# waiwnf/pilotguru

Hardware: AMD Instinct MI355X
Metric: frames/sec ORB extract+match, 1080p @ 2000 kp/frame (higher is better)
Workload: dtype u8

## Files before the change

pilotguru_amd/csrc/describe.hip:

```cpp
#include "pgorb_internal.h"

struct PgGauss7 { int k0, k1, k2, k3; };
constexpr PgGauss7 PG_G7 = {18, 34, 49, 55};

#define DH_N 37

struct PgDescTab { uint32_t mom[5 * 64]; uint32_t btab[3 * 64 * 4]; int8_t pat[64 * 4 * 4]; };
constexpr PgDescTab pg_make_desc_tab()
{
    constexpr int umax[16] = {15, 15, 15, 15, 14, 14, 14, 13, 13, 12, 11, 10, 9, 8, 6, 3};
    constexpr int8_t p[256 * 4] = {
#include "orb_pattern31.inc"
    };
    constexpr int K[7] = {PG_G7.k0, PG_G7.k1, PG_G7.k2, PG_G7.k3, PG_G7.k2, PG_G7.k1, PG_G7.k0};
    PgDescTab t = {};
    for (int r = 0; r < 31; r++)
        for (int q = 0; q < 9; q++) {
            const int vy = r - 15, dmax = umax[vy < 0 ? -vy : vy];
            uint32_t wu = 0;
            for (int k = 0; k < 4; k++) {
                const int ux = 4 * (q + 1) + k - 21;
                if ((ux < 0 ? -ux : ux) <= dmax) wu |= (uint32_t)(ux + 16) << (8 * k);
            }
            t.mom[r * 9 + q] = wu;
        }
    for (int cb = 0; cb < 3; cb++)
        for (int l = 0; l < 64; l++)
            for (int j = 0; j < 16; j++) {
                const int k = 16 * (l >> 4) + j, n = 16 * cb + (l & 15), d = k - n;
                const uint32_t v = (d >= 0 && d <= 6 && n < DH_N) ? (uint32_t)K[d] : 0u;
                t.btab[(cb * 64 + l) * 4 + j / 4] |= v << (8 * (j % 4));
            }
    for (int l = 0; l < 64; l++)
        for (int r = 0; r < 4; r++)
            for (int k = 0; k < 4; k++) t.pat[(l * 4 + r) * 4 + k] = p[(64 * r + l) * 4 + k];
    return t;
}
__device__ static const __attribute__((aligned(16))) PgDescTab pg_desc_tab = pg_make_desc_tab();

#define DW_R 21
#define DW_N 43
#define DW_PITCH 48
#define DH_PITCH 40
#define DB_PITCH 40

__device__ __forceinline__ int pg_reflect101(int p, int n)
{
    if (n == 1) return 0;
    while (p < 0 || p >= n) p = (p < 0) ? -p : 2 * (n - 1) - p;
    return p;
}

__device__ __forceinline__ float pg_fast_atan2(float y, float x)
{
    const float scale = (float)(180 / 3.1415926535897932384626433832795);
    const float p1 = 0.9997878412794807f * scale, p3 = -0.3258083974640975f * scale;
    const float p5 = 0.1555786518463281f * scale, p7 = -0.04432655554792128f * scale;
    const float eps = (float)2.2204460492503131e-16;
    const float ax = fabsf(x), ay = fabsf(y);
    float a, c, c2;
    if (ax >= ay) {
        c = __fdiv_rn(ay, __fadd_rn(ax, eps));
        c2 = __fmul_rn(c, c);
        a = __fmul_rn(__fadd_rn(__fmul_rn(__fadd_rn(__fmul_rn(__fadd_rn(__fmul_rn(p7, c2), p5), c2), p3), c2), p1), c);
    } else {
        c = __fdiv_rn(ax, __fadd_rn(ay, eps));
        c2 = __fmul_rn(c, c);
        a = __fsub_rn(90.f, __fmul_rn(__fadd_rn(__fmul_rn(__fadd_rn(__fmul_rn(__fadd_rn(__fmul_rn(p7, c2), p5), c2), p3), c2), p1), c));
    }
    if (x < 0) a = __fsub_rn(180.f, a);
    if (y < 0) a = __fsub_rn(360.f, a);
    return a;
}

__device__ __forceinline__ void pg_sincos_f(float angle, float* s_out, float* c_out)
{
    const double INV_PIO2 = 0.63661977236758138243;
    const double PIO2_HI = 1.57079632673412561417e+00;
    const double PIO2_LO = 6.07710050650619224932e-11;
    const double x = (double)angle;
    const double kd = floor(__dadd_rn(__dmul_rn(x, INV_PIO2), 0.5));
    const double r = __dsub_rn(__dsub_rn(x, __dmul_rn(kd, PIO2_HI)), __dmul_rn(kd, PIO2_LO));
    const double r2 = __dmul_rn(r, r);
    double ps = -1.0 / 355687428096000.0;
    ps = __dadd_rn(__dmul_rn(ps, r2), 1.0 / 1307674368000.0);
    ps = __dsub_rn(__dmul_rn(ps, r2), 1.0 / 6227020800.0);
    ps = __dadd_rn(__dmul_rn(ps, r2), 1.0 / 39916800.0);
    ps = __dsub_rn(__dmul_rn(ps, r2), 1.0 / 362880.0);
    ps = __dadd_rn(__dmul_rn(ps, r2), 1.0 / 5040.0);
    ps = __dsub_rn(__dmul_rn(ps, r2), 1.0 / 120.0);
    ps = __dadd_rn(__dmul_rn(ps, r2), 1.0 / 6.0);
    const double sn = __dsub_rn(r, __dmul_rn(__dmul_rn(r, r2), ps));
    double pc = -1.0 / 6402373705728000.0;
    pc = __dadd_rn(__dmul_rn(pc, r2), 1.0 / 20922789888000.0);
    pc = __dsub_rn(__dmul_rn(pc, r2), 1.0 / 87178291200.0);
    pc = __dadd_rn(__dmul_rn(pc, r2), 1.0 / 479001600.0);
    pc = __dsub_rn(__dmul_rn(pc, r2), 1.0 / 3628800.0);
    pc = __dadd_rn(__dmul_rn(pc, r2), 1.0 / 40320.0);
    pc = __dsub_rn(__dmul_rn(pc, r2), 1.0 / 720.0);
    pc = __dadd_rn(__dmul_rn(pc, r2), 1.0 / 24.0);
    pc = __dsub_rn(__dmul_rn(pc, r2), 0.5);
    const double cs = __dadd_rn(1.0, __dmul_rn(r2, pc));
    const int k = (int)((long long)kd & 3);
    const double s = (k == 0) ? sn : (k == 1) ? cs : (k == 2) ? -sn : -cs;
    const double c = (k == 0) ? cs : (k == 1) ? -sn : (k == 2) ? -cs : sn;
    *s_out = (float)s;
    *c_out = (float)c;
}

__device__ __forceinline__ int pg_wave_sum(int x)
{
    int v = x;
    v += __builtin_amdgcn_update_dpp(0, v, 0x111, 0xf, 0xf, true);
    v += __builtin_amdgcn_update_dpp(0, v, 0x112, 0xf, 0xf, true);
    v += __builtin_amdgcn_update_dpp(0, v, 0x114, 0xf, 0xf, true);
    v += __builtin_amdgcn_update_dpp(0, v, 0x118, 0xf, 0xf, true);
    v += __builtin_amdgcn_update_dpp(0, v, 0x142, 0xa, 0xf, false);
    v += __builtin_amdgcn_update_dpp(0, v, 0x143, 0xc, 0xf, false);
    return __builtin_amdgcn_readlane(v, 63);
}


typedef __attribute__((address_space(1))) const void* pg_gptr_t;
typedef __attribute__((address_space(3))) void* pg_lptr_t;
typedef unsigned short pg_us2 __attribute__((ext_vector_type(2)));
typedef int pg_v4i __attribute__((ext_vector_type(4)));
#define PG_GLOBAL __attribute__((address_space(1)))
typedef PG_GLOBAL const uint8_t* pg_gbytes_t;

__device__ __forceinline__ int pg_blur_at(const uint32_t* hT, int Y, int X, bool tieEven)
{
    constexpr PgGauss7 G = PG_G7;
    const pg_us2 K01 = {(unsigned short)G.k0, (unsigned short)G.k1}, K23 = {(unsigned short)G.k2, (unsigned short)G.k3},
                 K45 = {(unsigned short)G.k2, (unsigned short)G.k1};
    const uint32_t* s = hT + (Y >> 1) * 40 + X;
    const uint32_t p0 = s[0], p1 = s[40], p2 = s[80], p3 = s[120];
    const uint32_t sh = (uint32_t)(Y & 1) << 4;
    const uint32_t a0 = __builtin_amdgcn_alignbit(p1, p0, sh), a1 = __builtin_amdgcn_alignbit(p2, p1, sh),
                   a2 = __builtin_amdgcn_alignbit(p3, p2, sh), last = (p3 >> sh) & 0xFFFFu;
    uint32_t C = __builtin_amdgcn_udot2(__builtin_bit_cast(pg_us2, a0), K01, (uint32_t)G.k0 * last, false);
    C = __builtin_amdgcn_udot2(__builtin_bit_cast(pg_us2, a1), K23, C, false);
    C = __builtin_amdgcn_udot2(__builtin_bit_cast(pg_us2, a2), K45, C, false);
    int v = (int)((C + 32768u) >> 16);
    if (tieEven && (C & 0xFFFFu) == 0x8000u) v &= ~1;
    return min(v, 255);
}

#define PG_WAVE_SYNC() do { __builtin_amdgcn_fence(__ATOMIC_RELEASE, "wavefront"); __builtin_amdgcn_wave_barrier(); \
                            __builtin_amdgcn_fence(__ATOMIC_ACQUIRE, "wavefront"); } while (0)

struct PgDescArgs {
    const int32_t* kpCount;  const PgSelRec* sel;  int64_t selFrame;  pgorb_keypoint* kps;
    uint8_t* desc;  int32_t* n_out;  int32_t nlevels, tieMode, cap_per_frame, slotBeg;
    int32_t slotEnd, writeTotal, slotsPerXcd, pad[5];
};
static_assert(sizeof(PgDescArgs) == 96 && sizeof(PgDescArgs) <= 128, "one s_load_dwordx16 + one s_load_dwordx8");

__global__ __launch_bounds__(64) void k_describe(const PgDescArgs KA)
{
    __shared__ __attribute__((aligned(16))) uint32_t hbuf[22 * DH_PITCH];
    uint8_t* raw = reinterpret_cast<uint8_t*>(hbuf);

    const int lane = threadIdx.x;
    const uint32_t frame = blockIdx.y;
    typedef int32_t pg_i32x16 __attribute__((ext_vector_type(16)));
    typedef uint32_t pg_u32x16 __attribute__((ext_vector_type(16)));
    typedef uint32_t pg_u32x8 __attribute__((ext_vector_type(8)));
    pg_gbytes_t tb = (pg_gbytes_t)(const void*)&pg_desc_tab;
    asm volatile("" : "+s"(tb));
    const uint32_t o4 = 4u * (uint32_t)lane, o16 = 16u * (uint32_t)lane;
    uint32_t mt[5];
#pragma unroll
    for (int it = 0; it < 5; it++) mt[it] = *(const PG_GLOBAL uint32_t*)(tb + (offsetof(PgDescTab, mom) + 256 * it) + o4);
    pg_v4i Bop[3];
#pragma unroll
    for (int cb = 0; cb < 3; cb++) Bop[cb] = *(const PG_GLOBAL pg_v4i*)(tb + (offsetof(PgDescTab, btab) + 1024 * cb) + o16);
    const pg_v4i pat = *(const PG_GLOBAL pg_v4i*)(tb + offsetof(PgDescTab, pat) + o16);
    pg_u32x16 a0;
    pg_u32x8 a1;
    asm volatile("s_load_dwordx16 %0, %2, 0x0\n\ts_load_dwordx8 %1, %2, 0x40\n\ts_waitcnt lgkmcnt(0)"
                 : "=&s"(a0), "=&s"(a1) : "s"(__builtin_amdgcn_kernarg_segment_ptr()) : "memory");
#define PG_A64(T, v, k) reinterpret_cast<T>((uintptr_t)(((uint64_t)(v)[(k) + 1] << 32) | (v)[k]))
    const int32_t* kpCount = PG_A64(const int32_t*, a0, 0);
    const PgSelRec* sel = PG_A64(const PgSelRec*, a0, 2);
    const int64_t selFrame = (int64_t)(((uint64_t)a0[5] << 32) | a0[4]);
    pgorb_keypoint* kps = PG_A64(pgorb_keypoint*, a0, 6);
    uint8_t* desc = PG_A64(uint8_t*, a0, 8);
    int32_t* n_out = PG_A64(int32_t*, a0, 10);
#undef PG_A64
    const int nlevels = (int)a0[12], tieMode = (int)a0[13], cap_per_frame = (int)a0[14], slotBeg = (int)a0[15];
    const int slotEnd = (int)a1[0], writeTotal = (int)a1[1], slotsPerXcd = (int)a1[2];
    const int slot = slotBeg + (int)(blockIdx.x & 7) * slotsPerXcd + (int)(blockIdx.x >> 3);
    const int32_t* kpc = kpCount + frame * PG_MAXL;
    const PgSelRec* recp = sel + ((int64_t)frame * selFrame + slot);
    pg_i32x16 kc;
    pg_u32x8 rec;
    asm volatile("s_load_dwordx16 %0, %2, 0x0\n\ts_load_dwordx8 %1, %3, 0x0\n\ts_waitcnt lgkmcnt(0)" : "=&s"(kc), "=&s"(rec) : "s"(kpc), "s"(recp) : "memory");
    if (slot >= slotEnd) return;
    const int l = (int)(rec[1] >> 16) & 15;
    int total = 0, before = 0;
#pragma unroll
    for (int q = 0; q < PG_MAXL; q++) {
        const int c = kc[q];
        if (q < l) before += c;
        total += c;
    }
    if (writeTotal && blockIdx.x == 0 && lane == 0) n_out[frame] = total;
    if (rec[1] == 0xFFFFFFFFu || l >= nlevels) return;
    const uint32_t cv = rec[0];
    const int idx = before + (int)(rec[1] & 0xFFFFu);
    const int Lpitch = (int)rec[2], Lw = (int)(rec[3] & 0xFFFFu), Lh = (int)(rec[3] >> 16);
    const uint8_t* img = reinterpret_cast<const uint8_t*>((uintptr_t)(((uint64_t)rec[5] << 32) | rec[4]));
    const float Lscale = __uint_as_float(rec[6]), LpatchSize = __uint_as_float(rec[7]);
    const int x = (int)(cv & 0xFFF) + PG_EDGE, y = (int)((cv >> 12) & 0xFFF) + PG_EDGE;
    const int resp = (int)(cv >> 24);
    const int w = Lw, h = Lh;

    const int x0 = x - DW_R, y0 = y - DW_R;
    if (x0 >= 0 && y0 >= 0 && x0 + DW_PITCH <= w && y + DW_R < h) {
        const int lr = lane / 3, lq = lane - 3 * lr;
        const uint8_t* g = img + (int64_t)(y0 + lr) * Lpitch + x0 + 16 * lq;
        if (lr < 21) {
            __builtin_amdgcn_global_load_lds((pg_gptr_t)g, (pg_lptr_t)raw, 16, 0, 0);
            __builtin_amdgcn_global_load_lds((pg_gptr_t)(g + 21 * (int64_t)Lpitch), (pg_lptr_t)(raw + 21 * DW_PITCH), 16, 0, 0);
            if (lr < 1)
                __builtin_amdgcn_global_load_lds((pg_gptr_t)(g + 42 * (int64_t)Lpitch), (pg_lptr_t)(raw + 42 * DW_PITCH), 16, 0, 0);
        }
        __builtin_amdgcn_s_waitcnt(0);
    } else {
        for (int i = lane; i < DW_N * DW_PITCH; i += 64) {
            const int r = i / DW_PITCH, c = i - r * DW_PITCH;
            raw[r * DW_PITCH + c] =
                img[(int64_t)pg_reflect101(y0 + r, h) * Lpitch + pg_reflect101(x0 + c, w)];
        }
    }
    PG_WAVE_SYNC();

    int m10 = 0, m01 = 0;
#pragma unroll
    for (int it = 0; it < 5; it++) {
        const int i = lane + 64 * it;
        if (i >= 31 * 9) break;
        const int r = i / 9, q = i - r * 9;
        const uint32_t val = *reinterpret_cast<const uint32_t*>(raw + (DW_R - 15 + r) * DW_PITCH + 4 * (q + 1));
        const uint32_t wm = ((mt[it] + 0x7F7F7F7Fu) >> 7) & 0x01010101u;
        const int sv = (int)__builtin_amdgcn_udot4(val, wm, 0u, false);
        m10 += (int)__builtin_amdgcn_udot4(val, mt[it], 0u, false) - 16 * sv;
        m01 += (r - 15) * sv;
    }
    m10 = pg_wave_sum(m10);
    m01 = pg_wave_sum(m01);
    const float angle = pg_fast_atan2((float)m01, (float)m10);

    uint32_t* hT = hbuf;
    {
        constexpr int cinit = 128 * (2 * (PG_G7.k0 + PG_G7.k1 + PG_G7.k2) + PG_G7.k3);
        pg_v4i Aop[3];
#pragma unroll
        for (int rb = 0; rb < 3; rb++) {
            Aop[rb] = *reinterpret_cast<const pg_v4i*>(raw + (16 * rb + (lane & 15)) * DW_PITCH + 16 * (lane >> 4));
            Aop[rb].x ^= (int)0x80808080; Aop[rb].y ^= (int)0x80808080; Aop[rb].z ^= (int)0x80808080; Aop[rb].w ^= (int)0x80808080;
        }
        PG_WAVE_SYNC();
#pragma unroll
        for (int rb = 0; rb < 3; rb++) {
            const int pair = 8 * rb + 2 * (lane >> 4);
#pragma unroll
            for (int cb = 0; cb < 3; cb++) {
                const pg_v4i acc = __builtin_amdgcn_mfma_i32_16x16x64_i8(Aop[rb], Bop[cb], pg_v4i{cinit, cinit, cinit, cinit}, 0, 0, 0);
                const int n = 16 * cb + (lane & 15);
                if (n < DH_PITCH) {
                    if (pair < 22) hT[pair * DH_PITCH + n] = (uint32_t)acc.x | ((uint32_t)acc.y << 16);
                    if (pair + 1 < 22) hT[(pair + 1) * DH_PITCH + n] = (uint32_t)acc.z | ((uint32_t)acc.w << 16);
                }
            }
        }
    }
    PG_WAVE_SYNC();
    const int wvec = w & ~3;

    const float factorPI = (float)(3.1415926535897932384626433832795 / 180.f);
    float a, b;
    pg_sincos_f(__fmul_rn(angle, factorPI), &b, &a);
    unsigned long long bits[4];
#pragma unroll
    for (int r = 0; r < 4; r++) {
        const uint32_t pw = (uint32_t)pat[r];
        const float px0 = (float)(int8_t)(pw & 0xFF), py0 = (float)(int8_t)((pw >> 8) & 0xFF);
        const float px1 = (float)(int8_t)((pw >> 16) & 0xFF), py1 = (float)(int8_t)(pw >> 24);
        const int r0 = __float2int_rn(__fadd_rn(__fmul_rn(px0, b), __fmul_rn(py0, a)));
        const int c0 = __float2int_rn(__fsub_rn(__fmul_rn(px0, a), __fmul_rn(py0, b)));
        const int r1 = __float2int_rn(__fadd_rn(__fmul_rn(px1, b), __fmul_rn(py1, a)));
        const int c1 = __float2int_rn(__fsub_rn(__fmul_rn(px1, a), __fmul_rn(py1, b)));
        const int t0 = pg_blur_at(hT, 18 + r0, 18 + c0, tieMode == 0 && x + c0 < wvec);
        const int t1 = pg_blur_at(hT, 18 + r1, 18 + c1, tieMode == 0 && x + c1 < wvec);
        bits[r] = __ballot(t0 < t1);
    }

    if (idx < cap_per_frame && lane == 0) {
        const int64_t o = (int64_t)frame * cap_per_frame + idx;
        unsigned long long* d = reinterpret_cast<unsigned long long*>(desc + o * 32);
        d[0] = bits[0]; d[1] = bits[1]; d[2] = bits[2]; d[3] = bits[3];
        pgorb_keypoint k;
        k.x = (l != 0) ? __fmul_rn((float)x, Lscale) : (float)x;
        k.y = (l != 0) ? __fmul_rn((float)y, Lscale) : (float)y;
        k.size = LpatchSize;
        k.angle = angle;
        k.response = (float)resp;
        k.octave = l;
        k.class_id = -1;
        kps[o] = k;
    }
}

static PgGauss7 pg_gauss7()
{
    float cf[7];
    double sum = 0;
    for (int i = 0; i < 7; i++) {
        const double xx = i - 3.0;
        cf[i] = (float)exp(-0.5 / (2.0 * 2.0) * xx * xx);
        sum += cf[i];
    }
    sum = 1. / sum;
    int K[7];
    for (int i = 0; i < 7; i++) {
        cf[i] = (float)(cf[i] * sum);
        K[i] = (int)lrint((double)(cf[i] * 256.f));
    }
    PgGauss7 g = {K[0], K[1], K[2], K[3]};
    return g;
}

bool pg_launch_describe(const PgPlan& P, int nframes, pgorb_keypoint* d_kps, uint8_t* d_desc,
                        int cap_per_frame, int32_t* d_n, hipStream_t s)
{
    return pg_launch_describe_levels(P, nframes, d_kps, d_desc, cap_per_frame, d_n, 0, P.nlevels, s);
}

bool pg_launch_describe_levels(const PgPlan& P, int nframes, pgorb_keypoint* d_kps, uint8_t* d_desc,
                               int cap_per_frame, int32_t* d_n, int levelBeg, int levelEnd, hipStream_t s)
{
    static const PgGauss7 G = pg_gauss7();
    static const bool tapsOk = G.k0 == PG_G7.k0 && G.k1 == PG_G7.k1 && G.k2 == PG_G7.k2 && G.k3 == PG_G7.k3;
    if (!tapsOk) return false;
    PgDescArgs KA = {};
    KA.kpCount = P.kpCount; KA.sel = reinterpret_cast<const PgSelRec*>(P.sel); KA.selFrame = P.selFrame;
    KA.kps = d_kps; KA.desc = d_desc; KA.n_out = d_n;
    KA.nlevels = P.nlevels; KA.tieMode = P.tieMode; KA.cap_per_frame = cap_per_frame;
    KA.slotBeg = (int)P.lvl[levelBeg].selOff;
    KA.slotEnd = (levelEnd < P.nlevels) ? (int)P.lvl[levelEnd].selOff : P.selTotal;
    KA.writeTotal = levelEnd == P.nlevels ? 1 : 0;
    dim3 grid((KA.slotEnd - KA.slotBeg + 7) & ~7, nframes), block(64);
    KA.slotsPerXcd = (int)(grid.x >> 3);
    hipLaunchKernelGGL(k_describe, grid, block, 0, s, KA);
    return true;
}

__global__ __launch_bounds__(256) void k_sincos_checksum(uint32_t first_bits, uint32_t count, unsigned long long* out)
{
    const uint32_t base = first_bits + blockIdx.x * count;
    unsigned long long acc = 0;
    for (uint32_t i = threadIdx.x; i < count; i += 256) {
        float s, c;
        pg_sincos_f(__uint_as_float(base + i), &s, &c);
        acc += ((unsigned long long)__float_as_uint(s) * 0x9E3779B1ull + __float_as_uint(c)) * (2ull * i + 1ull);
    }
    __shared__ unsigned long long red[256];
    red[threadIdx.x] = acc;
    __syncthreads();
    for (int st = 128; st > 0; st >>= 1) {
        if ((int)threadIdx.x < st) red[threadIdx.x] += red[threadIdx.x + st];
        __syncthreads();
    }
    if (threadIdx.x == 0) out[blockIdx.x] = red[0];
}

extern "C" int pgorb_debug_sincos_checksum(uint32_t first_bits, uint32_t count, int nblocks, unsigned long long* out)
{
    if (!out || nblocks < 1 || count < 1) return PGORB_E_ARG;
    unsigned long long* d = nullptr;
// ... 7 lines not shown
```

pilotguru_amd/csrc/match.hip:

```cpp
#include "pgorb_internal.h"

#define MT_T 64
#define MT_TILE 256

__device__ __forceinline__ int pg_hamming256(const uint4& a0, const uint4& a1, const uint4& b0, const uint4& b1)
{
    return __popc(a0.x ^ b0.x) + __popc(a0.y ^ b0.y) + __popc(a0.z ^ b0.z) + __popc(a0.w ^ b0.w) +
           __popc(a1.x ^ b1.x) + __popc(a1.y ^ b1.y) + __popc(a1.z ^ b1.z) + __popc(a1.w ^ b1.w);
}

__device__ __forceinline__ void stage_tile(uint4* tile, const uint8_t* b, int j0, int nb, int tid, int nthreads)
{
    const int cnt = min(MT_TILE, nb - j0);
    const uint4* src = reinterpret_cast<const uint4*>(b + (int64_t)j0 * 32);
    for (int i = tid; i < 2 * cnt; i += nthreads) tile[i] = src[i];
}

__global__ __launch_bounds__(MT_T) void k_hamming_matrix(const uint8_t* __restrict__ a, int na,
                                                          const uint8_t* __restrict__ b, int nb,
                                                          uint16_t* __restrict__ out)
{
    __shared__ uint4 tile[2 * MT_TILE];
    const int i = blockIdx.x * MT_T + threadIdx.x;
    uint4 q0 = make_uint4(0, 0, 0, 0), q1 = q0;
    if (i < na) {
        q0 = reinterpret_cast<const uint4*>(a + (int64_t)i * 32)[0];
        q1 = reinterpret_cast<const uint4*>(a + (int64_t)i * 32)[1];
    }
    for (int j0 = blockIdx.y * MT_TILE; j0 < nb; j0 += gridDim.y * MT_TILE) {
        __syncthreads();
        stage_tile(tile, b, j0, nb, threadIdx.x, MT_T);
        __syncthreads();
        const int cnt = min(MT_TILE, nb - j0);
        if (i < na)
            for (int j = 0; j < cnt; j++)
                out[(int64_t)i * nb + j0 + j] = (uint16_t)pg_hamming256(q0, q1, tile[2 * j], tile[2 * j + 1]);
    }
}

typedef int pg_v4i __attribute__((ext_vector_type(4)));
typedef int pg_v8i __attribute__((ext_vector_type(8)));
typedef float pg_v4f __attribute__((ext_vector_type(4)));
typedef __attribute__((address_space(1))) const void* pg_gptr_t;
typedef __attribute__((address_space(3))) void* pg_lptr_t;

#define MX_BLOCK_BYTES 2048
#define MX_TILE_BLOCKS 8
#ifndef MX_TILE_BLOCKS_WIDE
#define MX_TILE_BLOCKS_WIDE 16
#endif
#define MX_WAVES 4
#define MX_IDX_BITS 13
#define MX_IDX_MASK ((1 << MX_IDX_BITS) - 1)
#define MX_MAX_TRAIN (1 << MX_IDX_BITS)
#define MX_SCALE 0x85858585

__device__ __forceinline__ uint32_t pg_fp4x8(uint32_t b)
{
    uint32_t x = (b | (b << 12)) & 0x000F000Fu;
    x = (x | (x << 6)) & 0x03030303u;
    x = (x | (x << 3)) & 0x11111111u;
    return (x << 3) ^ 0xAAAAAAAAu;
}

__device__ __forceinline__ pg_v4i pg_fp4x32(uint32_t bits32)
{
    pg_v4i v;
    v.x = (int)pg_fp4x8(bits32 & 0xFFu); v.y = (int)pg_fp4x8((bits32 >> 8) & 0xFFu);
    v.z = (int)pg_fp4x8((bits32 >> 16) & 0xFFu); v.w = (int)pg_fp4x8(bits32 >> 24);
    return v;
}

__global__ __launch_bounds__(128) void k_expand_trains(const uint8_t* __restrict__ tdesc, const int32_t* __restrict__ n,
                                                        int cap, const int32_t* __restrict__ pt, int nb_single,
                                                        int blocksPerPair, uint8_t* __restrict__ xt)
{
    const int p = blockIdx.y, tb = blockIdx.x;
    const int ft = pt ? pt[p] : 0;
    const int nb = pt ? min(n[ft], cap) : nb_single;
    if (16 * tb >= nb) return;
    const int s = threadIdx.x >> 6, l = threadIdx.x & 63;
    const int idx = 16 * tb + (l & 15);
    pg_v4i v = {0, 0, 0, 0};
    if (idx < nb) {
        const uint32_t* src = reinterpret_cast<const uint32_t*>(tdesc + ((int64_t)ft * cap + idx) * 32);
        v = pg_fp4x32(src[4 * s + (l >> 4)]);
    }
    *reinterpret_cast<pg_v4i*>(xt + ((int64_t)p * blocksPerPair + tb) * MX_BLOCK_BYTES + threadIdx.x * 16) = v;
}

__device__ __forceinline__ float pg_med3(float a, float b, float c) { return __builtin_amdgcn_fmed3f(a, b, c); }

__device__ __forceinline__ void mx_block(const pg_v4i (&B)[2], const pg_v4i (&A)[4][2], const pg_v4f kq, pg_v4f (&acc)[4])
{
#pragma unroll
    for (int s = 0; s < 2; s++) {
        const pg_v8i b8 = {B[s].x, B[s].y, B[s].z, B[s].w, 0, 0, 0, 0};
#pragma unroll
        for (int a = 0; a < 4; a++) {
            const pg_v8i a8 = {A[a][s].x, A[a][s].y, A[a][s].z, A[a][s].w, 0, 0, 0, 0};
            acc[a] = __builtin_amdgcn_mfma_scale_f32_16x16x128_f8f6f4(a8, b8, s == 0 ? kq : acc[a], 4, 4, 0, MX_SCALE, 0, MX_SCALE);
        }
    }
}

__device__ __forceinline__ void mx_load(const uint8_t* blockLane, pg_v4i (&B)[2])
{
#pragma unroll
    for (int s = 0; s < 2; s++) B[s] = *reinterpret_cast<const pg_v4i*>(blockLane + s * 1024);
}

template <bool MASK>
__device__ __forceinline__ void mx_update(const pg_v4f (&acc)[4], bool valid, float (&k1)[4][4], float (&k2)[4][4])
{
#pragma unroll
    for (int a = 0; a < 4; a++)
#pragma unroll
        for (int r = 0; r < 4; r++) {
            float key = acc[a][r];
            if (MASK) key = valid ? key : -1.f;
            k2[a][r] = pg_med3(k1[a][r], k2[a][r], key);
            k1[a][r] = pg_med3(k1[a][r], key, __builtin_inff());
        }
}

__device__ __forceinline__ void mx_update2(const pg_v4f (&accA)[4], const pg_v4f (&accB)[4], float (&k1)[4][4], float (&k2)[4][4])
{
#pragma unroll
    for (int a = 0; a < 4; a++)
#pragma unroll
        for (int r = 0; r < 4; r++) {
            const float x = accA[a][r], y = accB[a][r];
            k2[a][r] = __builtin_fmaxf(pg_med3(k1[a][r], x, y), k2[a][r]);
            k1[a][r] = __builtin_fmaxf(__builtin_fmaxf(k1[a][r], x), y);
        }
}

template <int WAVES, bool RAW>
__global__ __launch_bounds__(64 * WAVES) void k_match_mfma(const uint8_t* __restrict__ qdesc, const uint8_t* __restrict__ xt,
                                                           const int32_t* __restrict__ n, int cap,
                                                           const int32_t* __restrict__ pq, const int32_t* __restrict__ pt,
                                                           int na_single, int nb_single, int blocksPerPair, int npairs,
                                                           int32_t* best_idx, uint16_t* best, uint16_t* second)
{
    constexpr int TB = (RAW && WAVES == 16) ? MX_TILE_BLOCKS_WIDE : MX_TILE_BLOCKS;
    constexpr int TILE_BYTES = TB * MX_BLOCK_BYTES, RAW_BYTES = TB * 16 * 32;
    constexpr int EXP_BYTES = (RAW ? 1 : 2) * TILE_BYTES + MX_BLOCK_BYTES;
    __shared__ __attribute__((aligned(16))) uint8_t tile[EXP_BYTES + (RAW ? 2 * RAW_BYTES : 0)];
    const int p = blockIdx.x, qblk = blockIdx.y;
    if (p >= npairs) return;
    const int fq = pq ? pq[p] : 0, ft = pt ? pt[p] : 0;
    const int na = pq ? min(n[fq], cap) : na_single, nb = pt ? min(n[ft], cap) : nb_single;
    if (qblk * 64 * WAVES >= na) return;
    const int lane = threadIdx.x & 63, wv = threadIdx.x >> 6;
    const int qbase = qblk * 64 * WAVES + wv * 64;
    const bool active = qbase < na;
    const uint8_t* qd = qdesc + (int64_t)fq * cap * 32;
    const int64_t o = (int64_t)p * cap;

    pg_v4i A[4][2];
    float k1[4][4], k2[4][4];
#pragma unroll
    for (int a = 0; a < 4; a++)
#pragma unroll
        for (int r = 0; r < 4; r++) { k1[a][r] = -1.f; k2[a][r] = -1.f; }

    const int nblocks = (nb + 15) >> 4;
    const uint8_t* xp = RAW ? xt + (int64_t)ft * cap * 32 : xt + (int64_t)p * blocksPerPair * MX_BLOCK_BYTES;
    uint8_t* rawBase = tile + EXP_BYTES;
    auto stage = [&](int t0, int buf) {
        if (RAW) {
            for (int c0 = 64 * wv; c0 < RAW_BYTES / 16; c0 += 64 * WAVES) {
                const int c = c0 + lane, d = t0 * 16 + (c >> 1);
                if (d < nb)
                    __builtin_amdgcn_global_load_lds((pg_gptr_t)(xp + (int64_t)d * 32 + (c & 1) * 16),
                                                     (pg_lptr_t)(rawBase + buf * RAW_BYTES + c0 * 16), 16, 0, 0);
            }
        } else {
            const int cnt = min(TB, nblocks - t0);
            for (int kb = wv; kb < cnt * (MX_BLOCK_BYTES / 1024); kb += WAVES)
                __builtin_amdgcn_global_load_lds((pg_gptr_t)(xp + (int64_t)t0 * MX_BLOCK_BYTES + kb * 1024 + lane * 16),
                                                 (pg_lptr_t)(tile + buf * TILE_BYTES + kb * 1024), 16, 0, 0);
        }
    };
    auto compute_tile = [&](const uint8_t* bl, int t0, int cnt) {
        float kc = (float)((256 << (MX_IDX_BITS - 1)) + MX_IDX_MASK - (t0 * 16 + (lane & 15)));
        const int cntFull = min(cnt, (nb >> 4) - t0);
        pg_v4i B0[2], B1[2];
        pg_v4f acc[4];
        mx_load(bl, B0);
        int blk = 0;
        for (; blk + 2 <= cntFull; blk += 2, kc -= 32.f) {
            mx_load(bl + (blk + 1) * MX_BLOCK_BYTES, B1);
            mx_block(B0, A, pg_v4f{kc, kc, kc, kc}, acc);
            pg_v4f accB[4];
            mx_block(B1, A, pg_v4f{kc - 16.f, kc - 16.f, kc - 16.f, kc - 16.f}, accB);
            mx_load(bl + (blk + 2) * MX_BLOCK_BYTES, B0);
            mx_update2(acc, accB, k1, k2);
        }
        if (blk < cntFull) {
            mx_load(bl + (blk + 1) * MX_BLOCK_BYTES, B1);
            mx_block(B0, A, pg_v4f{kc, kc, kc, kc}, acc);
            mx_update<false>(acc, true, k1, k2);
            blk++; kc -= 16.f;
            if (blk < cnt) {
                mx_block(B1, A, pg_v4f{kc, kc, kc, kc}, acc);
                mx_update<true>(acc, (t0 + blk) * 16 + (lane & 15) < nb, k1, k2);
            }
        } else if (blk < cnt) {
            mx_block(B0, A, pg_v4f{kc, kc, kc, kc}, acc);
            mx_update<true>(acc, (t0 + blk) * 16 + (lane & 15) < nb, k1, k2);
        }
    };
    if (nblocks > 0) stage(0, 0);
#pragma unroll
    for (int a = 0; a < 4; a++) {
        const int q = qbase + 16 * a + (lane & 15);
        const uint32_t* src = reinterpret_cast<const uint32_t*>(qd + (int64_t)q * 32) + (lane >> 4);
#pragma unroll
        for (int s = 0; s < 2; s++) {
            A[a][s] = pg_v4i{0, 0, 0, 0};
            if (q < na) A[a][s] = pg_fp4x32(src[4 * s]);
        }
    }
    int buf = 0;
    for (int t0 = 0; t0 < nblocks; t0 += TB, buf ^= 1) {
        const int cnt = min(TB, nblocks - t0);
        __builtin_amdgcn_s_waitcnt(0);
        __syncthreads();
        if (!RAW && t0 + TB < nblocks) stage(t0 + TB, buf ^ 1);
        if (RAW) {
            const uint32_t* raw32 = reinterpret_cast<const uint32_t*>(rawBase + buf * RAW_BYTES);
            for (int e = threadIdx.x; e < TILE_BYTES / 16; e += 64 * WAVES) {
                const int l = e & 63, s = (e >> 6) & 1, blk = e >> 7;
                *reinterpret_cast<pg_v4i*>(tile + e * 16) = pg_fp4x32(raw32[(blk * 16 + (l & 15)) * 8 + 4 * s + (l >> 4)]);
            }
            __syncthreads();
            if (t0 + TB < nblocks) stage(t0 + TB, buf ^ 1);
        }
        if (!active) continue;
        compute_tile(tile + (RAW ? 0 : buf * TILE_BYTES) + lane * 16, t0, cnt);
    }
    if (!active) return;
#pragma unroll
    for (int a = 0; a < 4; a++)
#pragma unroll
        for (int r = 0; r < 4; r++) {
            int m1 = (int)k1[a][r], m2 = (int)k2[a][r];
#pragma unroll
            for (int m = 1; m < 16; m <<= 1) {
                const int o1 = __shfl_xor(m1, m), o2 = __shfl_xor(m2, m);
                const int hi = max(m1, o1);
                m2 = max(min(m1, o1), max(m2, o2));
                m1 = hi;
            }
            const int q = qbase + 16 * a + 4 * (lane >> 4) + r;
            if ((lane & 15) == 0 && q < na) {
                best_idx[o + q] = m1 >= 0 ? (int32_t)(MX_IDX_MASK - (m1 & MX_IDX_MASK)) : -1;
                best[o + q] = m1 >= 0 ? (uint16_t)(256 - (m1 >> MX_IDX_BITS)) : (uint16_t)65535;
                second[o + q] = m2 >= 0 ? (uint16_t)(256 - (m2 >> MX_IDX_BITS)) : (uint16_t)65535;
            }
        }
}

#define MT_WAVES 4
#define MT_SLICE_TILE 128

#define MT_IDX_BITS 20

__device__ __forceinline__ void best2_scan(const uint8_t* a, int na, const uint8_t* b, int nb,
                                           int32_t* best_idx, uint16_t* best, uint16_t* second,
                                           uint4* tiles, unsigned* part)
{
    const int lane = threadIdx.x & 63, wv = threadIdx.x >> 6;
    const int i = blockIdx.x * MT_T + lane;
    uint4 q0 = make_uint4(0, 0, 0, 0), q1 = q0;
    if (i < na) {
        q0 = reinterpret_cast<const uint4*>(a + (int64_t)i * 32)[0];
        q1 = reinterpret_cast<const uint4*>(a + (int64_t)i * 32)[1];
    }
    const int per = (nb + MT_WAVES - 1) / MT_WAVES;
    const int jb = wv * per, je = min(jb + per, nb);
    uint4* tile = tiles + wv * 2 * MT_SLICE_TILE;
    unsigned k1 = 0xFFFFFFFFu, k2 = 0xFFFFFFFFu;
    for (int j0 = jb; j0 < je; j0 += MT_SLICE_TILE) {
        const int cnt = min(MT_SLICE_TILE, je - j0);
        const uint4* src = reinterpret_cast<const uint4*>(b + (int64_t)j0 * 32);
        __builtin_amdgcn_wave_barrier();
        for (int k = lane; k < 2 * cnt; k += 64) tile[k] = src[k];
        __builtin_amdgcn_fence(__ATOMIC_RELEASE, "wavefront");
        __builtin_amdgcn_wave_barrier();
        __builtin_amdgcn_fence(__ATOMIC_ACQUIRE, "wavefront");
        for (int j = 0; j < cnt; j++) {
            const unsigned d = (unsigned)pg_hamming256(q0, q1, tile[2 * j], tile[2 * j + 1]);
            const unsigned key = (d << MT_IDX_BITS) | (unsigned)(j0 + j);
            k2 = min(k2, max(k1, key));
            k1 = min(k1, key);
        }
    }
    part[(wv * 64 + lane) * 2 + 0] = k1;
    part[(wv * 64 + lane) * 2 + 1] = k2;
    __syncthreads();
    if (wv == 0 && i < na) {
        unsigned m1 = 0xFFFFFFFFu, m2 = 0xFFFFFFFFu;
#pragma unroll
        for (int w = 0; w < 2 * MT_WAVES; w++) {
            const unsigned key = part[(w >> 1) * 128 + lane * 2 + (w & 1)];
            m2 = min(m2, max(m1, key));
            m1 = min(m1, key);
        }
        best_idx[i] = (m1 == 0xFFFFFFFFu) ? -1 : (int32_t)(m1 & ((1u << MT_IDX_BITS) - 1));
        best[i] = (m1 == 0xFFFFFFFFu) ? (uint16_t)65535 : (uint16_t)(m1 >> MT_IDX_BITS);
        second[i] = (m2 == 0xFFFFFFFFu) ? (uint16_t)65535 : (uint16_t)(m2 >> MT_IDX_BITS);
    }
}

__global__ __launch_bounds__(MT_T * MT_WAVES) void k_hamming_best2(const uint8_t* __restrict__ a, int na,
                                                         const uint8_t* __restrict__ b, int nb,
                                                         int32_t* best_idx, uint16_t* best, uint16_t* second)
{
    __shared__ uint4 tiles[MT_WAVES * 2 * MT_SLICE_TILE];
    __shared__ unsigned part[MT_WAVES * 64 * 2];
    best2_scan(a, na, b, nb, best_idx, best, second, tiles, part);
}

__global__ __launch_bounds__(MT_T * MT_WAVES) void k_match_batch(const uint8_t* __restrict__ desc,
                                                       const int32_t* __restrict__ n, int cap,
                                                       const int32_t* __restrict__ pq,
                                                       const int32_t* __restrict__ pt,
                                                       int32_t* best_idx, uint16_t* best, uint16_t* second)
{
    __shared__ uint4 tiles[MT_WAVES * 2 * MT_SLICE_TILE];
    __shared__ unsigned part[MT_WAVES * 64 * 2];
    const int p = blockIdx.y;
    const int fq = pq[p], ft = pt[p];
    const int na = min(n[fq], cap), nb = min(n[ft], cap);
    if ((int)blockIdx.x * MT_T >= na) return;
    const int64_t o = (int64_t)p * cap;
    best2_scan(desc + (int64_t)fq * cap * 32, na, desc + (int64_t)ft * cap * 32, nb,
               best_idx + o, best + o, second + o, tiles, part);
// ... 85 lines not shown
```

Baseline: 100,800.

## Share one MFMA blur band matrix, fuse moment reductions, defer level-count prefix

Restructures the describe kernel. The horizontal blur MFMA now uses a single banded B matrix with the input A operand shifted per column block, which cuts B-table registers and loads. The LDS row-sum buffer grows to 24x48 so stores need no bounds checks. The two wave reductions share one permlane32 swap. Moment loops run unconditionally because zero-weight tail tasks read inside the window. The per-level keypoint counts move from a scalar x16 load to a per-lane vector load, with a DPP prefix sum computed late to hide latency. The cost is more VGPRs for the 9 A operands and a larger LDS footprint, which a static assert keeps within 32 waves per CU.

```diff
diff --git a/pilotguru_amd/csrc/describe.hip b/pilotguru_amd/csrc/describe.hip
--- a/pilotguru_amd/csrc/describe.hip
+++ b/pilotguru_amd/csrc/describe.hip
@@ -5,7 +5,7 @@
 
 #define DH_N 37
 
-struct PgDescTab { uint32_t mom[5 * 64]; uint32_t btab[3 * 64 * 4]; int8_t pat[64 * 4 * 4]; };
+struct PgDescTab { uint32_t mom[5 * 64]; uint32_t btab[64 * 4]; int8_t pat[64 * 4 * 4]; };
 constexpr PgDescTab pg_make_desc_tab()
 {
     constexpr int umax[16] = {15, 15, 15, 15, 14, 14, 14, 13, 13, 12, 11, 10, 9, 8, 6, 3};
@@ -24,25 +24,33 @@
             }
             t.mom[r * 9 + q] = wu;
         }
-    for (int cb = 0; cb < 3; cb++)
-        for (int l = 0; l < 64; l++)
-            for (int j = 0; j < 16; j++) {
-                const int k = 16 * (l >> 4) + j, n = 16 * cb + (l & 15), d = k - n;
-                const uint32_t v = (d >= 0 && d <= 6 && n < DH_N) ? (uint32_t)K[d] : 0u;
-                t.btab[(cb * 64 + l) * 4 + j / 4] |= v << (8 * (j % 4));
-            }
+    for (int l = 0; l < 64; l++)
+        for (int j = 0; j < 16; j++) {
+            const int k = 16 * (l >> 4) + j, n = l & 15, d = k - n;
+            const uint32_t v = (d >= 0 && d <= 6) ? (uint32_t)K[d] : 0u;
+            t.btab[l * 4 + j / 4] |= v << (8 * (j % 4));
+        }
     for (int l = 0; l < 64; l++)
         for (int r = 0; r < 4; r++)
             for (int k = 0; k < 4; k++) t.pat[(l * 4 + r) * 4 + k] = p[(64 * r + l) * 4 + k];
     return t;
 }
+constexpr bool pg_mom_tail_is_zero()
+{
+    const PgDescTab t = pg_make_desc_tab();
+    for (int i = 31 * 9; i < 5 * 64; i++)
+        if (t.mom[i]) return false;
+    return true;
+}
+static_assert(pg_mom_tail_is_zero(), "the moment rounds run unconditionally: tasks past 31 * 9 must weigh nothing");
 __device__ static const __attribute__((aligned(16))) PgDescTab pg_desc_tab = pg_make_desc_tab();
 
 #define DW_R 21
 #define DW_N 43
 #define DW_PITCH 48
-#define DH_PITCH 40
-#define DB_PITCH 40
+#define DH_PAIRS 24
+#define DH_PITCH 48
+#define DH_LDS_MAX (163840 / 32 / 1280 * 1280)
 
 __device__ __forceinline__ int pg_reflect101(int p, int n)
 {
@@ -108,16 +116,23 @@
     *c_out = (float)c;
 }
 
-__device__ __forceinline__ int pg_wave_sum(int x)
-{
-    int v = x;
+__device__ __forceinline__ int pg_row_sum(int v)
+{
     v += __builtin_amdgcn_update_dpp(0, v, 0x111, 0xf, 0xf, true);
     v += __builtin_amdgcn_update_dpp(0, v, 0x112, 0xf, 0xf, true);
     v += __builtin_amdgcn_update_dpp(0, v, 0x114, 0xf, 0xf, true);
     v += __builtin_amdgcn_update_dpp(0, v, 0x118, 0xf, 0xf, true);
+    return v;
+}
+
+__device__ __forceinline__ void pg_wave_sum2(int& a, int& b)
+{
+    typedef unsigned pg_u2 __attribute__((ext_vector_type(2)));
+    const pg_u2 sw = __builtin_amdgcn_permlane32_swap((unsigned)a, (unsigned)b, false, false);
+    int v = pg_row_sum((int)(sw.x + sw.y));
     v += __builtin_amdgcn_update_dpp(0, v, 0x142, 0xa, 0xf, false);
-    v += __builtin_amdgcn_update_dpp(0, v, 0x143, 0xc, 0xf, false);
-    return __builtin_amdgcn_readlane(v, 63);
+    a = __builtin_amdgcn_readlane(v, 31);
+    b = __builtin_amdgcn_readlane(v, 63);
 }
 
 
@@ -133,8 +148,8 @@
     constexpr PgGauss7 G = PG_G7;
     const pg_us2 K01 = {(unsigned short)G.k0, (unsigned short)G.k1}, K23 = {(unsigned short)G.k2, (unsigned short)G.k3},
                  K45 = {(unsigned short)G.k2, (unsigned short)G.k1};
-    const uint32_t* s = hT + (Y >> 1) * 40 + X;
-    const uint32_t p0 = s[0], p1 = s[40], p2 = s[80], p3 = s[120];
+    const uint32_t* s = hT + (Y >> 1) * DH_PITCH + X;
+    const uint32_t p0 = s[0], p1 = s[DH_PITCH], p2 = s[2 * DH_PITCH], p3 = s[3 * DH_PITCH];
     const uint32_t sh = (uint32_t)(Y & 1) << 4;
     const uint32_t a0 = __builtin_amdgcn_alignbit(p1, p0, sh), a1 = __builtin_amdgcn_alignbit(p2, p1, sh),
                    a2 = __builtin_amdgcn_alignbit(p3, p2, sh), last = (p3 >> sh) & 0xFFFFu;
@@ -158,12 +173,12 @@
 
 __global__ __launch_bounds__(64) void k_describe(const PgDescArgs KA)
 {
-    __shared__ __attribute__((aligned(16))) uint32_t hbuf[22 * DH_PITCH];
+    __shared__ __attribute__((aligned(16))) uint32_t hbuf[DH_PAIRS * DH_PITCH];
+    static_assert(sizeof(hbuf) <= DH_LDS_MAX, "the row sums must leave room for 32 waves per CU");
     uint8_t* raw = reinterpret_cast<uint8_t*>(hbuf);
 
     const int lane = threadIdx.x;
     const uint32_t frame = blockIdx.y;
-    typedef int32_t pg_i32x16 __attribute__((ext_vector_type(16)));
     typedef uint32_t pg_u32x16 __attribute__((ext_vector_type(16)));
     typedef uint32_t pg_u32x8 __attribute__((ext_vector_type(8)));
     pg_gbytes_t tb = (pg_gbytes_t)(const void*)&pg_desc_tab;
@@ -172,9 +187,7 @@
     uint32_t mt[5];
 #pragma unroll
     for (int it = 0; it < 5; it++) mt[it] = *(const PG_GLOBAL uint32_t*)(tb + (offsetof(PgDescTab, mom) + 256 * it) + o4);
-    pg_v4i Bop[3];
-#pragma unroll
-    for (int cb = 0; cb < 3; cb++) Bop[cb] = *(const PG_GLOBAL pg_v4i*)(tb + (offsetof(PgDescTab, btab) + 1024 * cb) + o16);
+    const pg_v4i Bop = *(const PG_GLOBAL pg_v4i*)(tb + offsetof(PgDescTab, btab) + o16);
     const pg_v4i pat = *(const PG_GLOBAL pg_v4i*)(tb + offsetof(PgDescTab, pat) + o16);
     pg_u32x16 a0;
     pg_u32x8 a1;
@@ -191,24 +204,22 @@
     const int nlevels = (int)a0[12], tieMode = (int)a0[13], cap_per_frame = (int)a0[14], slotBeg = (int)a0[15];
     const int slotEnd = (int)a1[0], writeTotal = (int)a1[1], slotsPerXcd = (int)a1[2];
     const int slot = slotBeg + (int)(blockIdx.x & 7) * slotsPerXcd + (int)(blockIdx.x >> 3);
+    static_assert(PG_MAXL == 16, "one count per lane of a DPP row");
     const int32_t* kpc = kpCount + frame * PG_MAXL;
+    int kcount = *(const PG_GLOBAL int32_t*)((pg_gbytes_t)(const void*)kpc + 4u * ((uint32_t)lane & 15u));
     const PgSelRec* recp = sel + ((int64_t)frame * selFrame + slot);
-    pg_i32x16 kc;
     pg_u32x8 rec;
-    asm volatile("s_load_dwordx16 %0, %2, 0x0\n\ts_load_dwordx8 %1, %3, 0x0\n\ts_waitcnt lgkmcnt(0)" : "=&s"(kc), "=&s"(rec) : "s"(kpc), "s"(recp) : "memory");
+    asm volatile("s_load_dwordx8 %0, %1, 0x0\n\ts_waitcnt lgkmcnt(0)" : "=&s"(rec) : "s"(recp) : "memory");
     if (slot >= slotEnd) return;
     const int l = (int)(rec[1] >> 16) & 15;
-    int total = 0, before = 0;
-#pragma unroll
-    for (int q = 0; q < PG_MAXL; q++) {
-        const int c = kc[q];
-        if (q < l) before += c;
-        total += c;
-    }
-    if (writeTotal && blockIdx.x == 0 && lane == 0) n_out[frame] = total;
+    if (writeTotal && blockIdx.x == 0) {
+        int total = 0;
+#pragma unroll
+        for (int q = 0; q < PG_MAXL; q++) total += kpc[q];
+        if (lane == 0) n_out[frame] = total;
+    }
     if (rec[1] == 0xFFFFFFFFu || l >= nlevels) return;
     const uint32_t cv = rec[0];
-    const int idx = before + (int)(rec[1] & 0xFFFFu);
     const int Lpitch = (int)rec[2], Lw = (int)(rec[3] & 0xFFFFu), Lh = (int)(rec[3] >> 16);
     const uint8_t* img = reinterpret_cast<const uint8_t*>((uintptr_t)(((uint64_t)rec[5] << 32) | rec[4]));
     const float Lscale = __uint_as_float(rec[6]), LpatchSize = __uint_as_float(rec[7]);
@@ -220,11 +231,13 @@
     if (x0 >= 0 && y0 >= 0 && x0 + DW_PITCH <= w && y + DW_R < h) {
         const int lr = lane / 3, lq = lane - 3 * lr;
         const uint8_t* g = img + (int64_t)(y0 + lr) * Lpitch + x0 + 16 * lq;
+        typedef __attribute__((address_space(3))) uint8_t* pg_lbytes_t;
+        const pg_lbytes_t lraw = (pg_lbytes_t)hbuf;
         if (lr < 21) {
-            __builtin_amdgcn_global_load_lds((pg_gptr_t)g, (pg_lptr_t)raw, 16, 0, 0);
-            __builtin_amdgcn_global_load_lds((pg_gptr_t)(g + 21 * (int64_t)Lpitch), (pg_lptr_t)(raw + 21 * DW_PITCH), 16, 0, 0);
+            __builtin_amdgcn_global_load_lds((pg_gptr_t)g, (pg_lptr_t)lraw, 16, 0, 0);
+            __builtin_amdgcn_global_load_lds((pg_gptr_t)(g + 21 * (int64_t)Lpitch), (pg_lptr_t)(lraw + 21 * DW_PITCH), 16, 0, 0);
             if (lr < 1)
-                __builtin_amdgcn_global_load_lds((pg_gptr_t)(g + 42 * (int64_t)Lpitch), (pg_lptr_t)(raw + 42 * DW_PITCH), 16, 0, 0);
+                __builtin_amdgcn_global_load_lds((pg_gptr_t)(g + 42 * (int64_t)Lpitch), (pg_lptr_t)(lraw + 42 * DW_PITCH), 16, 0, 0);
         }
         __builtin_amdgcn_s_waitcnt(0);
     } else {
@@ -236,43 +249,48 @@
     }
     PG_WAVE_SYNC();
 
+    static_assert(DW_R - 15 + (63 + 64 * 4) / 9 < DW_N, "the zero-weight tasks read inside the window");
     int m10 = 0, m01 = 0;
+    const int r0 = lane / 9, q0 = lane - 9 * r0;
+    const uint8_t* mrow = raw + (DW_R - 15 + r0) * DW_PITCH + 4 * (q0 + 1);
 #pragma unroll
     for (int it = 0; it < 5; it++) {
-        const int i = lane + 64 * it;
-        if (i >= 31 * 9) break;
-        const int r = i / 9, q = i - r * 9;
-        const uint32_t val = *reinterpret_cast<const uint32_t*>(raw + (DW_R - 15 + r) * DW_PITCH + 4 * (q + 1));
+        const bool carry = q0 + it >= 9;
+        const int v = r0 + 7 * it - 15 + (carry ? 1 : 0);
+        const uint32_t val = *reinterpret_cast<const uint32_t*>(mrow + it * (7 * DW_PITCH + 4) + (carry ? DW_PITCH - 36 : 0));
         const uint32_t wm = ((mt[it] + 0x7F7F7F7Fu) >> 7) & 0x01010101u;
         const int sv = (int)__builtin_amdgcn_udot4(val, wm, 0u, false);
         m10 += (int)__builtin_amdgcn_udot4(val, mt[it], 0u, false) - 16 * sv;
-        m01 += (r - 15) * sv;
-    }
-    m10 = pg_wave_sum(m10);
-    m01 = pg_wave_sum(m01);
+        m01 += v * sv;
+    }
+    pg_wave_sum2(m10, m01);
     const float angle = pg_fast_atan2((float)m01, (float)m10);
 
     uint32_t* hT = hbuf;
     {
         constexpr int cinit = 128 * (2 * (PG_G7.k0 + PG_G7.k1 + PG_G7.k2) + PG_G7.k3);
-        pg_v4i Aop[3];
+        static_assert(47 * DW_PITCH + 16 * (3 + 2) + 16 <= (int)sizeof(hbuf), "row operands stay inside the wave's buffer");
+        pg_v4i Aop[3][3];
+#pragma unroll
+        for (int rb = 0; rb < 3; rb++)
+#pragma unroll
+            for (int cb = 0; cb < 3; cb++) {
+                pg_v4i& A = Aop[rb][cb];
+                A = *reinterpret_cast<const pg_v4i*>(raw + (16 * rb + (lane & 15)) * DW_PITCH + 16 * (lane >> 4) + 16 * cb);
+                A.x ^= (int)0x80808080; A.y ^= (int)0x80808080; A.z ^= (int)0x80808080; A.w ^= (int)0x80808080;
+            }
+        PG_WAVE_SYNC();
 #pragma unroll
         for (int rb = 0; rb < 3; rb++) {
-            Aop[rb] = *reinterpret_cast<const pg_v4i*>(raw + (16 * rb + (lane & 15)) * DW_PITCH + 16 * (lane >> 4));
-            Aop[rb].x ^= (int)0x80808080; Aop[rb].y ^= (int)0x80808080; Aop[rb].z ^= (int)0x80808080; Aop[rb].w ^= (int)0x80808080;
-        }
-        PG_WAVE_SYNC();
-#pragma unroll
-        for (int rb = 0; rb < 3; rb++) {
-            const int pair = 8 * rb + 2 * (lane >> 4);
+            pg_v4i acc[3];
+#pragma unroll
+            for (int cb = 0; cb < 3; cb++)
+                acc[cb] = __builtin_amdgcn_mfma_i32_16x16x64_i8(Aop[rb][cb], Bop, pg_v4i{cinit, cinit, cinit, cinit}, 0, 0, 0);
+            uint32_t* o = hT + (8 * rb + 2 * (lane >> 4)) * DH_PITCH + (lane & 15);
 #pragma unroll
             for (int cb = 0; cb < 3; cb++) {
-                const pg_v4i acc = __builtin_amdgcn_mfma_i32_16x16x64_i8(Aop[rb], Bop[cb], pg_v4i{cinit, cinit, cinit, cinit}, 0, 0, 0);
-                const int n = 16 * cb + (lane & 15);
-                if (n < DH_PITCH) {
-                    if (pair < 22) hT[pair * DH_PITCH + n] = (uint32_t)acc.x | ((uint32_t)acc.y << 16);
-                    if (pair + 1 < 22) hT[(pair + 1) * DH_PITCH + n] = (uint32_t)acc.z | ((uint32_t)acc.w << 16);
-                }
+                o[16 * cb] = (uint32_t)acc[cb].x | ((uint32_t)acc[cb].y << 16);
+                o[16 * cb + DH_PITCH] = (uint32_t)acc[cb].z | ((uint32_t)acc[cb].w << 16);
             }
         }
     }
@@ -297,6 +315,9 @@
         bits[r] = __ballot(t0 < t1);
     }
 
+    asm volatile("" : "+v"(kcount));
+    const int before = __builtin_amdgcn_readlane(pg_row_sum(lane < l ? kcount : 0), 15);
+    const int idx = before + (int)(rec[1] & 0xFFFFu);
     if (idx < cap_per_frame && lane == 0) {
         const int64_t o = (int64_t)frame * cap_per_frame + idx;
         unsigned long long* d = reinterpret_cast<unsigned long long*>(desc + o * 32);
```

Measured after the change: 101,600 (median of 6 runs). Within noise of the previous version (+0.8%).

## Double-buffer expanded train tiles and overlap expansion with MFMA compute

Applied to the files above, without the earlier changes.

The RAW path now keeps two expanded tile buffers. The next tile is expanded after computing the current one, which removes the extra barrier between expansion and compute, and global staging runs two tiles ahead. The fp4 expansion switches from bit-twiddling to v_perm byte lookups. The final 16-lane reduction uses DPP row operations instead of shuffles. The changes also add readfirstlane scalarisation and earlier B-block loads to hide LDS latency. In exchange, shared memory use grows and the read-ahead relies on slack buffers past the tile end.

```diff
diff --git a/pilotguru_amd/csrc/match.hip b/pilotguru_amd/csrc/match.hip
--- a/pilotguru_amd/csrc/match.hip
+++ b/pilotguru_amd/csrc/match.hip
@@ -55,19 +55,12 @@
 #define MX_MAX_TRAIN (1 << MX_IDX_BITS)
 #define MX_SCALE 0x85858585
 
-__device__ __forceinline__ uint32_t pg_fp4x8(uint32_t b)
-{
-    uint32_t x = (b | (b << 12)) & 0x000F000Fu;
-    x = (x | (x << 6)) & 0x03030303u;
-    x = (x | (x << 3)) & 0x11111111u;
-    return (x << 3) ^ 0xAAAAAAAAu;
-}
-
 __device__ __forceinline__ pg_v4i pg_fp4x32(uint32_t bits32)
 {
+    const uint32_t T = 0x222AA2AAu;
     pg_v4i v;
-    v.x = (int)pg_fp4x8(bits32 & 0xFFu); v.y = (int)pg_fp4x8((bits32 >> 8) & 0xFFu);
-    v.z = (int)pg_fp4x8((bits32 >> 16) & 0xFFu); v.w = (int)pg_fp4x8(bits32 >> 24);
+    v.x = (int)__builtin_amdgcn_perm(T, T, bits32 & 0x03030303u); v.y = (int)__builtin_amdgcn_perm(T, T, (bits32 >> 2) & 0x03030303u);
+    v.z = (int)__builtin_amdgcn_perm(T, T, (bits32 >> 4) & 0x03030303u); v.w = (int)__builtin_amdgcn_perm(T, T, (bits32 >> 6) & 0x03030303u);
     return v;
 }
 
@@ -124,16 +117,26 @@
         }
 }
 
+template <int A0, int A1>
 __device__ __forceinline__ void mx_update2(const pg_v4f (&accA)[4], const pg_v4f (&accB)[4], float (&k1)[4][4], float (&k2)[4][4])
 {
 #pragma unroll
-    for (int a = 0; a < 4; a++)
+    for (int a = A0; a < A1; a++)
 #pragma unroll
         for (int r = 0; r < 4; r++) {
             const float x = accA[a][r], y = accB[a][r];
             k2[a][r] = __builtin_fmaxf(pg_med3(k1[a][r], x, y), k2[a][r]);
             k1[a][r] = __builtin_fmaxf(__builtin_fmaxf(k1[a][r], x), y);
         }
+}
+
+template <int CTRL>
+__device__ __forceinline__ void mx_merge(int& m1, int& m2)
+{
+    const int o1 = __builtin_amdgcn_update_dpp(0, m1, CTRL, 0xF, 0xF, false), o2 = __builtin_amdgcn_update_dpp(0, m2, CTRL, 0xF, 0xF, false);
+    const int hi = max(m1, o1);
+    m2 = max(min(m1, o1), max(m2, o2));
+    m1 = hi;
 }
 
 template <int WAVES, bool RAW>
@@ -145,14 +148,16 @@
 {
     constexpr int TB = (RAW && WAVES == 16) ? MX_TILE_BLOCKS_WIDE : MX_TILE_BLOCKS;
     constexpr int TILE_BYTES = TB * MX_BLOCK_BYTES, RAW_BYTES = TB * 16 * 32;
-    constexpr int EXP_BYTES = (RAW ? 1 : 2) * TILE_BYTES + MX_BLOCK_BYTES;
-    __shared__ __attribute__((aligned(16))) uint8_t tile[EXP_BYTES + (RAW ? 2 * RAW_BYTES : 0)];
+    constexpr int EXP_BYTES = 2 * TILE_BYTES;
+    static_assert(2 * RAW_BYTES >= 2 * MX_BLOCK_BYTES, "the raw tiles are the read-ahead slack");
+    __shared__ __attribute__((aligned(16))) uint8_t tile[EXP_BYTES + (RAW ? 2 * RAW_BYTES : 2 * MX_BLOCK_BYTES)];
     const int p = blockIdx.x, qblk = blockIdx.y;
     if (p >= npairs) return;
-    const int fq = pq ? pq[p] : 0, ft = pt ? pt[p] : 0;
-    const int na = pq ? min(n[fq], cap) : na_single, nb = pt ? min(n[ft], cap) : nb_single;
+    const int fq = __builtin_amdgcn_readfirstlane(pq ? pq[p] : 0), ft = __builtin_amdgcn_readfirstlane(pt ? pt[p] : 0);
+    const int na = __builtin_amdgcn_readfirstlane(pq ? min(n[fq], cap) : na_single);
+    const int nb = __builtin_amdgcn_readfirstlane(pt ? min(n[ft], cap) : nb_single);
     if (qblk * 64 * WAVES >= na) return;
-    const int lane = threadIdx.x & 63, wv = threadIdx.x >> 6;
+    const int lane = threadIdx.x & 63, wv = __builtin_amdgcn_readfirstlane(threadIdx.x >> 6);
     const int qbase = qblk * 64 * WAVES + wv * 64;
     const bool active = qbase < na;
     const uint8_t* qd = qdesc + (int64_t)fq * cap * 32;
@@ -183,33 +188,43 @@
                                                  (pg_lptr_t)(tile + buf * TILE_BYTES + kb * 1024), 16, 0, 0);
         }
     };
-    auto compute_tile = [&](const uint8_t* bl, int t0, int cnt) {
-        float kc = (float)((256 << (MX_IDX_BITS - 1)) + MX_IDX_MASK - (t0 * 16 + (lane & 15)));
+    auto expand = [&](int rbuf, int ebuf) {
+        const uint32_t* raw32 = reinterpret_cast<const uint32_t*>(rawBase + rbuf * RAW_BYTES);
+        int e0 = threadIdx.x;
+        asm volatile("" : "+v"(e0));
+        for (int e = e0; e < TILE_BYTES / 16; e += 64 * WAVES) {
+            const int l = e & 63, s = (e >> 6) & 1, blk = e >> 7;
+            *reinterpret_cast<pg_v4i*>(tile + ebuf * TILE_BYTES + e * 16) = pg_fp4x32(raw32[(blk * 16 + (l & 15)) * 8 + 4 * s + (l >> 4)]);
+        }
+    };
+    auto compute_tile = [&](const uint8_t* bl, int col, int t0, int cnt) {
+        float kc = (float)((256 << (MX_IDX_BITS - 1)) + MX_IDX_MASK - (t0 * 16 + col));
         const int cntFull = min(cnt, (nb >> 4) - t0);
         pg_v4i B0[2], B1[2];
         pg_v4f acc[4];
         mx_load(bl, B0);
+        mx_load(bl + MX_BLOCK_BYTES, B1);
         int blk = 0;
         for (; blk + 2 <= cntFull; blk += 2, kc -= 32.f) {
-            mx_load(bl + (blk + 1) * MX_BLOCK_BYTES, B1);
             mx_block(B0, A, pg_v4f{kc, kc, kc, kc}, acc);
+            mx_load(bl + (blk + 2) * MX_BLOCK_BYTES, B0);
             pg_v4f accB[4];
             mx_block(B1, A, pg_v4f{kc - 16.f, kc - 16.f, kc - 16.f, kc - 16.f}, accB);
-            mx_load(bl + (blk + 2) * MX_BLOCK_BYTES, B0);
-            mx_update2(acc, accB, k1, k2);
+            mx_update2<0, 2>(acc, accB, k1, k2);
+            mx_load(bl + (blk + 3) * MX_BLOCK_BYTES, B1);
+            mx_update2<2, 4>(acc, accB, k1, k2);
         }
         if (blk < cntFull) {
-            mx_load(bl + (blk + 1) * MX_BLOCK_BYTES, B1);
             mx_block(B0, A, pg_v4f{kc, kc, kc, kc}, acc);
             mx_update<false>(acc, true, k1, k2);
             blk++; kc -= 16.f;
             if (blk < cnt) {
                 mx_block(B1, A, pg_v4f{kc, kc, kc, kc}, acc);
-                mx_update<true>(acc, (t0 + blk) * 16 + (lane & 15) < nb, k1, k2);
+                mx_update<true>(acc, (t0 + blk) * 16 + col < nb, k1, k2);
             }
         } else if (blk < cnt) {
             mx_block(B0, A, pg_v4f{kc, kc, kc, kc}, acc);
-            mx_update<true>(acc, (t0 + blk) * 16 + (lane & 15) < nb, k1, k2);
+            mx_update<true>(acc, (t0 + blk) * 16 + col < nb, k1, k2);
         }
     };
     if (nblocks > 0) stage(0, 0);
@@ -222,40 +237,35 @@
             A[a][s] = pg_v4i{0, 0, 0, 0};
             if (q < na) A[a][s] = pg_fp4x32(src[4 * s]);
         }
+    }
+    if (RAW && nblocks > 0) {
+        __builtin_amdgcn_s_waitcnt(0);
+        __syncthreads();
+        expand(0, 0);
+        if (TB < nblocks) stage(TB, 1);
     }
     int buf = 0;
     for (int t0 = 0; t0 < nblocks; t0 += TB, buf ^= 1) {
         const int cnt = min(TB, nblocks - t0);
         __builtin_amdgcn_s_waitcnt(0);
         __syncthreads();
-        if (!RAW && t0 + TB < nblocks) stage(t0 + TB, buf ^ 1);
-        if (RAW) {
-            const uint32_t* raw32 = reinterpret_cast<const uint32_t*>(rawBase + buf * RAW_BYTES);
-            for (int e = threadIdx.x; e < TILE_BYTES / 16; e += 64 * WAVES) {
-                const int l = e & 63, s = (e >> 6) & 1, blk = e >> 7;
-                *reinterpret_cast<pg_v4i*>(tile + e * 16) = pg_fp4x32(raw32[(blk * 16 + (l & 15)) * 8 + 4 * s + (l >> 4)]);
-            }
-            __syncthreads();
-            if (t0 + TB < nblocks) stage(t0 + TB, buf ^ 1);
-        }
-        if (!active) continue;
-        compute_tile(tile + (RAW ? 0 : buf * TILE_BYTES) + lane * 16, t0, cnt);
+        if (t0 + (RAW ? 2 : 1) * TB < nblocks) stage(t0 + (RAW ? 2 : 1) * TB, RAW ? buf : buf ^ 1);
+        int ln = lane;
+        asm volatile("" : "+v"(ln));
+        if (active) compute_tile(tile + buf * TILE_BYTES + ln * 16, ln & 15, t0, cnt);
+        if (RAW && t0 + TB < nblocks) expand(buf ^ 1, buf ^ 1);
     }
     if (!active) return;
+    const int el = __builtin_amdgcn_mbcnt_hi(~0u, __builtin_amdgcn_mbcnt_lo(~0u, 0u));
 #pragma unroll
     for (int a = 0; a < 4; a++)
 #pragma unroll
         for (int r = 0; r < 4; r++) {
             int m1 = (int)k1[a][r], m2 = (int)k2[a][r];
-#pragma unroll
-            for (int m = 1; m < 16; m <<= 1) {
-                const int o1 = __shfl_xor(m1, m), o2 = __shfl_xor(m2, m);
-                const int hi = max(m1, o1);
-                m2 = max(min(m1, o1), max(m2, o2));
-                m1 = hi;
-            }
-            const int q = qbase + 16 * a + 4 * (lane >> 4) + r;
-            if ((lane & 15) == 0 && q < na) {
+            mx_merge<0xB1>(m1, m2); mx_merge<0x4E>(m1, m2);
+            mx_merge<0x141>(m1, m2); mx_merge<0x140>(m1, m2);
+            const int q = qbase + 16 * a + 4 * (el >> 4) + r;
+            if ((el & 15) == 0 && q < na) {
                 best_idx[o + q] = m1 >= 0 ? (int32_t)(MX_IDX_MASK - (m1 & MX_IDX_MASK)) : -1;
                 best[o + q] = m1 >= 0 ? (uint16_t)(256 - (m1 >> MX_IDX_BITS)) : (uint16_t)65535;
                 second[o + q] = m2 >= 0 ? (uint16_t)(256 - (m2 >> MX_IDX_BITS)) : (uint16_t)65535;
```

Result: no change. 99860 before, 100,100 after (median of 6 runs) (+0.2%).
